# comfy-creator/Comfy-Gen-Server

Hardware: AMD Instinct MI355X
Metric: images/sec (whole node) + sec/image, SDXL 1024 20-step Euler-a at 1/2/4/8 MI355X (higher is better)
Workload: dtype bf16; 1 GPU; model=sdxl-base, global_batch=8, seq_len=16384, resolution=1024, sampler_steps=20, sampler=euler_ancestral, unet_batch_per_gpu=16, parallelism=dp1, pipelined=True

## Files before the change

### comfy_gen_server_amd/_native.py

```python
from __future__ import annotations

import ctypes
import glob
import os
import threading

_HERE = os.path.dirname(os.path.abspath(__file__))
LIB_DIR = os.path.join(_HERE, "lib")
_lock = threading.Lock()
_kernels = None
_kernels_err = None


def kernel_lib_path() -> str:
    return os.environ.get("CGS_KERNELS_SO") or os.path.join(LIB_DIR, "libcgs_kernels.so")


def load_kernels():
    global _kernels, _kernels_err
    if _kernels is not None or _kernels_err is not None:
        return _kernels
    with _lock:
        if _kernels is not None or _kernels_err is not None:
            return _kernels
        path = kernel_lib_path()
        if not os.path.exists(path):
            _kernels_err = f"{path} not built (run python build_native.py)"
            return None
        try:
            import torch
            lib = ctypes.CDLL(path, mode=ctypes.RTLD_GLOBAL)
            _declare(lib)
            _kernels = lib
        except OSError as e:
            _kernels_err = str(e)
            _kernels = None
    return _kernels


def kernels_error():
    return _kernels_err


_P = ctypes.c_void_p
_I = ctypes.c_int
_L = ctypes.c_longlong
_F = ctypes.c_float

KERNEL_SIGNATURES = {
    "cgs_groupnorm_nhwc_ws": [_P, _P, _P, _P, _P, _P, _I, _I, _I, _I, _F, _I, _I, _P],
    "cgs_groupnorm_workspace": [_I, _I, _I],
    "cgs_groupnorm_nhwc_dual": [_P, _P, _I, _P, _P, _P, _P, _P, _I, _I, _I, _I, _F, _I, _I, _P],
    "cgs_layernorm": [_P, _P, _P, _P, _I, _I, _F, _I, _P],
    "cgs_flash_attn_fwd": [_P, _P, _P, _P,
                           _I, _I, _I, _I, _I,
                           _L, _L, _L,
                           _L, _L, _L,
                           _L, _L, _L,
                           _L, _L, _L,
                           _F, _P, _I, _P],
    "cgs_flash_attn_fwd_v": [_P, _P, _P, _P, _I, _I, _I, _I, _I, _L, _L, _L, _L, _L, _L, _L, _L, _L, _L, _L, _L, _F,
                             _I, _P],
    "cgs_flash_attn_fwd_bias": [_P, _P, _P, _P, _I, _I, _I, _I, _I, _L, _L, _L, _L, _L, _L, _L, _L, _L, _L, _L, _L,
                                _F, _P, _P, _I, _P, _P],
    "cgs_flash_attn_fwd_mask": [_P, _P, _P, _P, _I, _I, _I, _I, _I, _L, _L, _L, _L, _L, _L, _L, _L, _L, _L, _L, _L,
                                _F, _P, _I, _L, _L, _L, _P, _I, _P],
    "cgs_flash_attn_fwd_lse": [_P, _P, _P, _P, _P, _I, _I, _I, _I, _I, _L, _L, _L, _L, _L, _L, _L, _L, _L, _L, _L, _L,
                               _F, _P],
    "cgs_gemm_bf16": [_P, _P, _P, _P, _P, _I, _I, _I, _L, _L, _L, _L, _I, _F, _P],
    "cgs_gemm_set_variant": [_I],
    "cgs_conv_set_variant": [_I],
    "cgs_attn_set_variant": [_I],
    "cgs_set_tile_group": [_I],
    "cgs_conv_set_tile_group": [_I],
    "cgs_dwconv_set_px": [_I],
    "cgs_affine_layernorm": [_P, _P, _P, _L, _F, _P, _P, _I, _I, _I, _F, _I, _P],
    "cgs_geglu": [_P, _P, _I, _I, _I, _P],
    "cgs_cfg_combine": [_P, _P, _P, _L, _F, _I, _P],
    "cgs_euler_step": [_P, _P, _P, _L, _F, _F, _F, _P],
    "cgs_timestep_embedding": [_P, _P, _I, _I, _F, _I, _P],
    "cgs_silu": [_P, _P, _L, _I, _P],
    "cgs_act": [_P, _P, _L, _I, _F, _I, _P],
    "cgs_upsample_nearest2x_nhwc": [_P, _P, _I, _I, _I, _I, _I, _P],
    "cgs_dwconv_nhwc": [_P, _P, _P, _P, _I, _I, _I, _I, _I, _I, _I, _P],
    "cgs_dwconv_ln_stats_nhwc": [_P, _P, _P, _P, _P, _I, _I, _I, _I, _I, _I, _F, _I, _P],
    "cgs_conv2d_nhwc": [_P, _P, _P, _P, _P, _I, _I, _I, _I, _I, _I, _I, _I, _I, _I, _I, _P],
    "cgs_fused_bias_act": [_P, _P, _P, _L, _I, _L, _F, _F, _I, _P],
    "cgs_upfirdn2d": [_P, _P, _P, _I, _I, _I, _I, _I, _I, _I, _I, _I, _I, _I, _I, _I, _I, _P],
    "cgs_resize": [_P, _P, _I, _I, _I, _I, _I, _I, _I, _I, _P],
    "cgs_lanczos_u8_h": [_P, _L, _L, _L, _L, _P, _I, _I, _I, _I, _I, _P, _P, _I, _I, _I, _P],
    "cgs_lanczos_u8_v": [_P, _I, _L, _L, _L, _L, _P, _I, _I, _I, _I, _P, _P, _I, _P],
    "cgs_bislerp": [_P, _P, _I, _I, _I, _I, _L, _L, _L, _L, _I, _I, _P, _P, _P, _I, _I, _P],
    "cgs_filter_sep": [_P, _P, _P, _P, _P, _I, _I, _I, _I, _I, _I, _I, _L, _L, _L, _L, _L, _L, _L, _L, _I, _F, _F, _F, _F,
                       _I, _P],
    "cgs_morph_box": [_P, _P, _P, _I, _I, _I, _I, _I, _L, _L, _L, _L, _L, _L, _L, _L, _I, _I, _I, _P],
    "cgs_canny_nms": [_P, _P, _P, _I, _I, _I, _F, _F, _P],
    "cgs_hysteresis_sweep": [_P, _I, _I, _I, _P, _P],
    "cgs_vq_nearest": [_P, _P, _P, _P, _I, _I, _I, _I, _P],
    "cgs_grn_nhwc": [_P, _P, _P, _P, _P, _I, _I, _I, _I, _P],
    "cgs_grn_stats": [_P, _P, _I, _I, _I, _I, _I, _P],
    "cgs_splitk_ws_bytes": [_I, _I, _I],
    "cgs_gemm_bf16_splitk": [_P, _P, _P, _P, _P, _P, _P, _I, _I, _I, _L, _L, _L, _L, _I, _F, _I, _I, _P, _L, _P],
    "cgs_grn_stats_gns": [_P, _P, _I, _I, _I, _P],
    "cgs_grn_apply_gns": [_P, _P, _P, _P, _P, _P, _I, _I, _I, _P],
    "cgs_gemm_bf16_gelu_gns": [_P, _P, _P, _P, _P, _P, _I, _I, _I, _L, _L, _L, _I, _P, _I, _P],
    "cgs_grn_scale_weight": [_P, _P, _P, _I, _I, _I, _I, _P, _P],
    "cgs_h2d_upload": [_P, _P, _L, _L, _I, _P],
    "cgs_gemm_f32": [_P, _P, _P, _P, _P, _I, _I, _I, _L, _L, _L, _L, _I, _F, _I, _I, _L, _L, _L, _P],
    "cgs_conv_f32": [_P, _P, _P, _P, _P, _P, _I, _I, _I, _I, _I, _I, _I, _I, _I, _I, _I, _I, _I, _P],
    "cgs_groupnorm_f32_ws": [_I, _I, _I],
    "cgs_groupnorm_f32": [_P, _P, _I, _P, _P, _P, _P, _P, _I, _I, _I, _I, _F, _I, _P],
    "cgs_layernorm_f32": [_P, _P, _P, _P, _L, _I, _F, _P],
    "cgs_softmax_rows": [_P, _P, _L, _I, _F, _I, _P],
    "cgs_gemm_bf16_w8": [_P, _P, _P, _P, _P, _I, _I, _I, _L, _L, _L, _L, _I, _F, _P],
    "cgs_gemm_bf16_v": [_P, _P, _P, _P, _P, _I, _I, _I, _L, _L, _L, _L, _I, _F, _I, _P],
    "cgs_conv2d_nhwc_v": [_P, _P, _I, _P, _P, _P, _P, _I, _I, _I, _I, _I, _I, _I, _I, _I, _I, _I, _I, _I, _P],
    "cgs_upconv_taps_nhwc": [_P, _P, _P, _P, _I, _I, _I, _I, _I, _P],
    "cgs_conv2d_nhwc_act": [_P, _P, _I, _P, _P, _P, _P, _I, _I, _I, _I, _I, _I, _I, _I, _I, _I, _I, _I, _I, _I, _F,
                            _P],
    "cgs_philox_randn": [_P, _I, _L, ctypes.c_ulonglong, _L, ctypes.c_ulonglong, _P, _F, _I, _P, _P],
    "cgs_euler_ancestral_philox": [_P, _P, _I, _L, _F, _F, _F, ctypes.c_ulonglong, _L, ctypes.c_ulonglong, _P, _P],
    "cgs_brownian_increment": [_P, _I, _L, ctypes.c_ulonglong, _L, ctypes.c_double, ctypes.c_double,
                               ctypes.c_double, ctypes.c_double, ctypes.c_double, _I, _F, _P, _P],
    "cgs_sampler_step_dev": [_P, _P, _P, _P, _I, _L, _F, _P, _I, _P, _P],
    "cgs_step_param": [_P, _I, _P, _I, _I, _P, _P],
    "cgs_step_advance": [_P, _P],
    "cgs_vae_out_u8": [_P, _P, _L, _P],
    "cgs_conv2d_nhwc_ex": [_P, _P, _I, _P, _P, _P, _P, _I, _I, _I, _I, _I, _I, _I, _I, _I, _I, _I, _I, _P],
    "cgs_region_accumulate": [_P, _P, _P, _I, _P, _I, _I, _I, _I, _I, _I, _I, _I, _I, _L, _L, _L, _L, _I, _L, _L,
                              _L, _L, _I, _F, _P],
    "cgs_region_normalize": [_P, _P, _P, _L, _I, _P],
    "cgs_clip_embed": [_P, _P, _P, _P, _I, _I, _I, _I, _I, _P],
    "cgs_pooled_gather": [_P, _P, _P, _I, _I, _I, _I, _P],
    "cgs_layernorm_stats": [_P, _P, _I, _I, _F, _I, _P],
    "cgs_gemm_bf16_lnfold": [_P, _P, _P, _P, _P, _P, _I, _I, _I, _L, _L, _L, _I, _P, _L, _P],
    "cgs_gemm_bf16_lnfold_v": [_P, _P, _P, _P, _P, _P, _I, _I, _I, _L, _L, _L, _I, _P, _L, _I, _P],
    "cgs_v7_ws_bytes": [_I, _I, _I],
    "cgs_v7_set_dbg": [_I],
    "cgs_v6_set_mode": [_I],
    "cgs_attn_set_prio": [_I],
    "cgs_gn_set_blocks": [_I],
    "cgs_conv_smalln_set_lds": [_I],
    "cgs_attn_set_kv2_rows": [_I],
    "cgs_grn_set_rows": [_I],
    "cgs_flash_attn_fwd_ks": [_P, _P, _P, _P, _I, _I, _I, _I, _L, _L, _L, _L, _L, _L, _L, _L, _F, _I, _P, _P, _P],
    "cgs_flash_attn_fwd_kv2": [_P, _P, _P, _P, _P, _P, _I, _I, _I, _I, _I, _L, _L, _L, _L, _L, _L, _L, _L, _L, _L, _L, _L, _F, _P],
    "cgs_conv2d_nhwc_gns": [_P, _P, _I, _P, _P, _P, _P, _I, _I, _I, _I, _I, _I, _I, _I, _I, _I, _I, _I, _P, _P],
    "cgs_groupnorm_band_stats": [_P, _P, _I, _P, _P, _P, _I, _I, _I, _I, _I, _P],
    "cgs_groupnorm_apply_stats": [_P, _P, _I, _P, _P, _P, _P, _P, _P, _I, _I, _I, _I, _I, _I, _P],
    "cgs_groupnorm_nhwc_part": [_P, _P, _P, _P, _P, _P, _P, _I, _I, _I, _I, _I, _F, _I, _I, _P],
    "cgs_groupnorm_nhwc_part_pld": [_P, _P, _P, _P, _P, _I, _P, _P, _I, _I, _I, _I, _I, _F, _I, _I, _P],
    "cgs_groupnorm_nhwc_ws_pld": [_P, _P, _P, _P, _P, _I, _P, _I, _I, _I, _I, _F, _I, _I, _P],
    "cgs_groupnorm_nhwc_dual_pld": [_P, _P, _I, _P, _P, _P, _P, _I, _P, _I, _I, _I, _I, _F, _I, _I, _P],
    "cgs_gemm_bf16_v7ws": [_P, _P, _P, _P, _P, _I, _I, _I, _L, _L, _L, _L, _I, _F, _P, _L, _P],
    "cgs_conv2d_nhwc_v7ws": [_P, _P, _I, _P, _P, _P, _P, _I, _I, _I, _I, _I, _I, _I, _I, _I, _I, _I, _I, _P, _L, _P],
    "cgs_fourier_filter": [_P, _P, _P, _I, _I, _I, _I, _L, _L, _L, _L, _L, _L, _L, _L, _I, _F, _I, _P],
    "cgs_tome_match": [_P, _P, _P, _P, _P, _I, _I, _I, _I, _L, _L, _L, _L, _I, _P],
    "cgs_grn_nhwc_v2": [_P, _P, _P, _P, _P, _I, _I, _I, _I, _I, _P],
    "cgs_grn_slices": [_I, _I, _I],
    "cgs_bgemm_f32": [_P, _P, _P, _I, _I, _I, _I, _L, _L, _L, _L, _L, _L, _L, _L, _F, _I, _I, _P],
    "cgs_softmax2_f32_bf16": [_P, _P, _L, _I, _L, _L, _P],
    "cgs_transpose_bf16": [_P, _P, _I, _I, _L, _L, _P],
    "cgs_abort_stream_capture": [_P],
    "cgs_channel_affine2": [_P, _P, _P, _L, _P, _I, _I, _I, _F, _I, _P],
    "cgs_gemm_bf16_w6": [_P, _P, _P, _P, _P, _P, _P, _I, _I, _I, _L, _L, _L, _L, _I, _F, _I, _I, _I, _I, _P],
    "cgs_gemm_w6_ok": [_I, _I, _I, _L, _L, _L, _L, _I, _I],
    "cgs_gemm_skinny_ws": [_P, _P, _P, _P, _P, _I, _I, _I, _L, _L, _L, _L, _I, _F, _P, _L, _P],
    "cgs_gemm_skinny_ws_bytes": [_I, _I, _I],
    "cgs_gemm_bf16_rowstats": [_P, _P, _P, _P, _P, _I, _I, _I, _L, _L, _L, _L, _I, _F, _P, _P],
    "cgs_gemm_bf16_rowstats_v": [_P, _P, _P, _P, _P, _I, _I, _I, _L, _L, _L, _L, _I, _F, _P, _I, _P],
    "cgs_ln_rs_from_partials": [_P, _P, _I, _I, _F, _P],
    "cgs_conv_v6_set_loader": [_I],
    "cgs_upconv_set_tile_group": [_I],
}


_RESTYPE = {"cgs_groupnorm_workspace": ctypes.c_longlong, "cgs_splitk_ws_bytes": ctypes.c_longlong, "cgs_groupnorm_f32_ws": ctypes.c_longlong, "cgs_grn_slices": ctypes.c_int, "cgs_v7_ws_bytes": ctypes.c_longlong, "cgs_gemm_skinny_ws_bytes": ctypes.c_longlong, "cgs_gemm_set_variant": None, "cgs_v7_set_dbg": None, "cgs_v6_set_mode": None, "cgs_attn_set_prio": None, "cgs_gn_set_blocks": None, "cgs_conv_smalln_set_lds": None, "cgs_attn_set_kv2_rows": None, "cgs_grn_set_rows": None,
            "cgs_conv_set_variant": None, "cgs_set_tile_group": None, "cgs_conv_set_tile_group": None, "cgs_dwconv_set_px": None, "cgs_upconv_set_tile_group": None,
            "cgs_attn_set_variant": None,
            "cgs_conv_v6_set_loader": None}


def _declare(lib):
    for name, argtypes in KERNEL_SIGNATURES.items():
        fn = getattr(lib, name, None)
        if fn is None:
            continue
        fn.argtypes = argtypes
        fn.restype = _RESTYPE.get(name, ctypes.c_int)


def has_kernel(name: str) -> bool:
    lib = load_kernels()
    return lib is not None and getattr(lib, name, None) is not None


_runtime = None
_runtime_err = None


def load_runtime():
    global _runtime, _runtime_err
    if _runtime is not None or _runtime_err is not None:
        return _runtime
    import importlib.util
    import sys
    cands = glob.glob(os.path.join(LIB_DIR, "_cgs_runtime*.so"))
    if not cands:
        _runtime_err = "_cgs_runtime not built"
        return None
    try:
        spec = importlib.util.spec_from_file_location("_cgs_runtime", cands[0])
        mod = importlib.util.module_from_spec(spec)
        spec.loader.exec_module(mod)
        sys.modules["_cgs_runtime"] = mod
        _runtime = mod
    except Exception as e:
        _runtime_err = str(e)
    return _runtime


def runtime_error():
    return _runtime_err
```

### comfy_gen_server_amd/csrc/kernels/norm.hip

```cpp
#include "common.h"

#define GN_THREADS 256
#define GN_MAX_CHUNKS_PER_LANE 4

static int g_gn_blocks = -1;
static int gn_blocks() {
  if (g_gn_blocks < 0) g_gn_blocks = getenv("CGS_GN_BLOCKS") ? atoi(getenv("CGS_GN_BLOCKS")) : 2048;
  return g_gn_blocks > 0 ? g_gn_blocks : 2048;
}
CGS_EXPORT void cgs_gn_set_blocks(int n) { g_gn_blocks = n; }

static inline int gn_pix_per_block(int N, int HW) {
  int target_blocks_per_n = (gn_blocks() + N - 1) / N;
  int ppb = (HW + target_blocks_per_n - 1) / target_blocks_per_n;
  if (ppb < 16) ppb = 16;
  if (N <= 4 && ppb < 64) ppb = 64;
  return ppb;
}

__device__ __forceinline__ const u16* gn_src(const u16* __restrict__ x, const u16* __restrict__ x2, int C, int C1,
                                             size_t pix, int c) {
  return c < C1 ? x + pix * C1 + c : x2 + pix * (size_t)(C - C1) + (c - C1);
}

template <int DT, int KM, int PK = 1>
__global__ __launch_bounds__(GN_THREADS) void gn_partial_kernel(const u16* __restrict__ x, const u16* __restrict__ x2,
                                                               int C1, float* __restrict__ part,
                                                               int HW, int C, int ppb, int nb, int CS) {
  constexpr int GN_UNROLL = 4;
  constexpr int LPG = 64 / PK;
  const int n = blockIdx.y;
  const int blk = blockIdx.x;
  const int c0 = blockIdx.z * CS;
  const int p0 = blk * ppb;
  const int p1 = min(HW, p0 + ppb);
  const int lane = threadIdx.x & 63;
  const int wave = threadIdx.x >> 6;
  const int lch = PK > 1 ? lane % LPG : lane;
  const int pg = PK > 1 ? lane / LPG : 0;
  const int nchunk = CS >> 3;
  const size_t pix0 = (size_t)n * HW;
  float s1[KM][8], s2[KM][8], sh[KM][8];
#pragma unroll
  for (int k = 0; k < KM; ++k) {
    int ch = lch + 64 * k;
    s16x8 v = {};
    if (ch < nchunk && p0 < p1) v = *reinterpret_cast<const s16x8*>(gn_src(x, x2, C, C1, pix0 + p0, c0 + ch * 8));
#pragma unroll
    for (int j = 0; j < 8; ++j) { sh[k][j] = cvt_in<DT>((u16)v[j]); s1[k][j] = 0.f; s2[k][j] = 0.f; }
  }
  int cnt = 0;
  for (int p = p0 + wave * PK + pg; p < p1; p += 4 * PK * GN_UNROLL) {
    s16x8 buf[GN_UNROLL][KM];
#pragma unroll
    for (int u = 0; u < GN_UNROLL; ++u) {
      const int pu = p + 4 * PK * u;
#pragma unroll
      for (int k = 0; k < KM; ++k) {
        int ch = lch + 64 * k;
        if (pu < p1 && ch < nchunk) buf[u][k] = *reinterpret_cast<const s16x8*>(gn_src(x, x2, C, C1, pix0 + pu, c0 + ch * 8));
      }
    }
#pragma unroll
    for (int u = 0; u < GN_UNROLL; ++u) {
      if (p + 4 * PK * u < p1) {
        cnt++;
#pragma unroll
        for (int k = 0; k < KM; ++k) {
          if (lch + 64 * k < nchunk) {
#pragma unroll
            for (int j = 0; j < 8; ++j) {
              float d = cvt_in<DT>((u16)buf[u][k][j]) - sh[k][j];
              s1[k][j] += d;
              s2[k][j] += d * d;
            }
          }
        }
      }
    }
  }
  if constexpr (PK > 1) {
#pragma unroll
    for (int off = LPG; off < 64; off <<= 1) {
      cnt += __shfl_xor(cnt, off);
#pragma unroll
      for (int j = 0; j < 8; ++j) {
        s1[0][j] += __shfl_xor(s1[0][j], off);
        s2[0][j] += __shfl_xor(s2[0][j], off);
      }
    }
  }
  extern __shared__ __attribute__((aligned(16))) float gn_smem[];
  float* lmean = gn_smem;
  float* lm2 = gn_smem + 4 * CS;
  __shared__ int lcnt[4];
  if (lane == 0) lcnt[wave] = cnt;
#pragma unroll
  for (int k = 0; k < KM; ++k) {
    int ch = lch + 64 * k;
    if (ch < nchunk && pg == 0) {
#pragma unroll
      for (int j = 0; j < 8; ++j) {
        float m = 0.f, m2 = 0.f;
        if (cnt > 0) {
          m = sh[k][j] + s1[k][j] / cnt;
          m2 = fmaxf(0.f, s2[k][j] - s1[k][j] * s1[k][j] / cnt);
        }
        lmean[wave * CS + ch * 8 + j] = m;
        lm2[wave * CS + ch * 8 + j] = m2;
      }
    }
  }
  __syncthreads();
  for (int c = threadIdx.x; c < CS; c += GN_THREADS) {
    float n_a = 0.f, mean = 0.f, m2 = 0.f;
    for (int w = 0; w < 4; ++w) {
      float n_b = (float)lcnt[w];
      if (n_b <= 0.f) continue;
      float mb = lmean[w * CS + c], m2b = lm2[w * CS + c];
      float nn = n_a + n_b;
      float d = mb - mean;
      mean += d * n_b / nn;
      m2 += m2b + d * d * n_a * n_b / nn;
      n_a = nn;
    }
    size_t o = (((size_t)n * nb + blk) * C + c0 + c) * 2;
    part[o] = mean;
    part[o + 1] = m2;
  }
}

__device__ __forceinline__ void chan_merge(float& na, float& ma, float& qa, float nb, float mb, float qb) {
  const float nn = na + nb;
  if (nn <= 0.f) return;
  const float d = mb - ma;
  const float f = nb / nn;
  ma += d * f;
  qa += qb + d * d * na * f;
  na = nn;
}

template <bool STATS_ONLY = false>
__global__ __launch_bounds__(256) void gn_finalize_kernel(const float* __restrict__ part, const void* __restrict__ gamma,
                                                         const void* __restrict__ beta, const void* __restrict__ pre_add,
                                                         float* __restrict__ ab, int HW, int C, int G, int ppb, int nb,
                                                         float eps, int wdt, int pld) {
  const int g = blockIdx.x;
  const int n = blockIdx.y;
  const int tid = threadIdx.x;
  const int Cg = C / G;
  const int items = Cg * nb;
  __shared__ float red[3][4];
  auto chan_shift = [&](int c) -> float {
    if (!pre_add) return 0.f;
    const size_t i = (size_t)n * pld + c;
    return (wdt == CGS_BF16) ? bf2f(((const u16*)pre_add)[i])
                             : (wdt == CGS_F16 ? h2f(((const u16*)pre_add)[i]) : ((const float*)pre_add)[i]);
  };
  float cnt = 0.f, mean = 0.f, m2 = 0.f;
  constexpr int U = 8;
  for (int it0 = tid; it0 < items; it0 += 256 * U) {
    float2 v[U];
    float nbv[U];
#pragma unroll
    for (int u = 0; u < U; ++u) {
      const int it = it0 + 256 * u;
      v[u] = make_float2(0.f, 0.f);
      nbv[u] = 0.f;
      if (it < items) {
        const int b = it / Cg, cc = it - b * Cg;
        const int c = g * Cg + cc;
        v[u] = *reinterpret_cast<const float2*>(part + (((size_t)n * nb + b) * C + c) * 2);
        v[u].x += chan_shift(c);
        nbv[u] = (float)(min(HW, b * ppb + ppb) - b * ppb);
      }
    }
#pragma unroll
    for (int u = 0; u < U; ++u) chan_merge(cnt, mean, m2, nbv[u], v[u].x, v[u].y);
  }
#pragma unroll
  for (int off = 32; off > 0; off >>= 1) {
    const float on = __shfl_xor(cnt, off), om = __shfl_xor(mean, off), oq = __shfl_xor(m2, off);
    chan_merge(cnt, mean, m2, on, om, oq);
  }
  if ((tid & 63) == 0) { red[0][tid >> 6] = cnt; red[1][tid >> 6] = mean; red[2][tid >> 6] = m2; }
  __syncthreads();
  cnt = red[0][0]; mean = red[1][0]; m2 = red[2][0];
#pragma unroll
  for (int w = 1; w < 4; ++w) chan_merge(cnt, mean, m2, red[0][w], red[1][w], red[2][w]);
  if constexpr (STATS_ONLY) {
    if (tid == 0) {
      ab[((size_t)n * G + g) * 2] = mean;
      ab[((size_t)n * G + g) * 2 + 1] = m2;
    }
    return;
  }
  const float var = m2 / fmaxf(cnt, 1.f);
  const float rstd = rsqrtf(fmaxf(var, 0.f) + eps);
  for (int cc = tid; cc < Cg; cc += 256) {
    int c = g * Cg + cc;
    float gm = 1.f, bt = 0.f;
    if (gamma) gm = (wdt == CGS_BF16) ? bf2f(((const u16*)gamma)[c]) : (wdt == CGS_F16 ? h2f(((const u16*)gamma)[c]) : ((const float*)gamma)[c]);
    if (beta) bt = (wdt == CGS_BF16) ? bf2f(((const u16*)beta)[c]) : (wdt == CGS_F16 ? h2f(((const u16*)beta)[c]) : ((const float*)beta)[c]);
    float a = rstd * gm;
    ab[((size_t)n * C + c) * 2] = a;
    ab[((size_t)n * C + c) * 2 + 1] = (chan_shift(c) - mean) * a + bt;
  }
}

template <int DT, bool SILU>
__global__ __launch_bounds__(256) void gn_apply_kernel(const u16* __restrict__ x, const u16* __restrict__ x2, int C1,
                                                      u16* __restrict__ y,
                                                      const float* __restrict__ ab, int rows_total, int rows_per_iter,
                                                      int HW, int C) {
  const int cpr = C >> 3;
  const int tid = blockIdx.x * blockDim.x + threadIdx.x;
  if (tid >= rows_per_iter * cpr) return;
  const int ch = tid % cpr;
  int cur_n = -1;
  float a[8], bb[8];
  auto coef = [&](int n) {
    if (n != cur_n) {
      cur_n = n;
      const float4* abp = reinterpret_cast<const float4*>(ab + ((size_t)n * C + ch * 8) * 2);
#pragma unroll
      for (int j = 0; j < 4; ++j) {
        float4 t = abp[j];
        a[2 * j] = t.x; bb[2 * j] = t.y; a[2 * j + 1] = t.z; bb[2 * j + 1] = t.w;
      }
    }
  };
  auto apply = [&](int row, const s16x8& v) {
    coef(row / HW);
    s16x8 o;
#pragma unroll
    for (int j = 0; j < 8; ++j) {
      float f = cvt_in<DT>((u16)v[j]) * a[j] + bb[j];
      if (SILU) f = silu_f(f);
      o[j] = (short)cvt_out<DT>(f);
    }
    reinterpret_cast<s16x8*>(y)[(size_t)row * cpr + ch] = o;
  };
  int row = tid / cpr;
  for (; row + rows_per_iter < rows_total; row += 2 * rows_per_iter) {
    const s16x8 v0 = *reinterpret_cast<const s16x8*>(gn_src(x, x2, C, C1, (size_t)row, ch * 8));
    const s16x8 v1 = *reinterpret_cast<const s16x8*>(gn_src(x, x2, C, C1, (size_t)(row + rows_per_iter), ch * 8));
    apply(row, v0);
    apply(row + rows_per_iter, v1);
  }
  if (row < rows_total) apply(row, *reinterpret_cast<const s16x8*>(gn_src(x, x2, C, C1, (size_t)row, ch * 8)));
}

template <int PV>
__global__ __launch_bounds__(256) void ln_rs_from_partials_kernel(const float* __restrict__ part, float* __restrict__ rs,
                                                                  int M, int P, float eps) {
  const int row = blockIdx.x * 256 + threadIdx.x;
  if (row >= M) return;
  float n, mean, m2;
  auto chan = [&](float vm, float vq) {
    const float nn = n + 80.f, d = vm - mean, f = 80.f / nn;
    mean += d * f;
    m2 += vq + d * d * n * f;
    n = nn;
  };
  if constexpr (PV > 0) {
    const float4* p = reinterpret_cast<const float4*>(part) + (long long)row * (P >> 1);
    float4 v[PV];
#pragma unroll
    for (int c = 0; c < PV; ++c) v[c] = 2 * c < P ? p[c] : float4{0.f, 0.f, 0.f, 0.f};
    n = 80.f, mean = v[0].x, m2 = v[0].y;
    chan(v[0].z, v[0].w);
#pragma unroll
    for (int c = 1; c < PV; ++c)
      if (2 * c < P) {
        chan(v[c].x, v[c].y);
        chan(v[c].z, v[c].w);
      }
  } else {
    const float2* p = reinterpret_cast<const float2*>(part) + (long long)row * P;
    n = 80.f, mean = p[0].x, m2 = p[0].y;
    for (int c = 1; c < P; ++c) chan(p[c].x, p[c].y);
  }
  reinterpret_cast<float2*>(rs)[row] = float2{mean, rsqrtf(m2 / n + eps)};
}

CGS_EXPORT int cgs_ln_rs_from_partials(const float* part, float* rs, int M, int P, float eps, hipStream_t stream) {
  if (M <= 0 || P <= 0) return (int)hipErrorInvalidValue;
  const unsigned grid = (unsigned)((M + 255) / 256);
  const bool vec = P % 2 == 0 && ((uintptr_t)part & 15) == 0;
  if (vec && P <= 8) ln_rs_from_partials_kernel<4><<<grid, 256, 0, stream>>>(part, rs, M, P, eps);
  else if (vec && P <= 16) ln_rs_from_partials_kernel<8><<<grid, 256, 0, stream>>>(part, rs, M, P, eps);
  else ln_rs_from_partials_kernel<0><<<grid, 256, 0, stream>>>(part, rs, M, P, eps);
  return (int)hipGetLastError();
}

CGS_EXPORT long long cgs_groupnorm_workspace(int N, int HW, int C) {
  int ppb = gn_pix_per_block(N, HW);
  int nb = (HW + ppb - 1) / ppb;
  return (long long)N * nb * C * 2 * 4 + (long long)N * C * 2 * 4 + 256;
}

static int gn_apply_launch(const void* x, const void* x2, int C1, void* y, const float* ab, int N, int HW, int C,
                           int silu, int dtype, hipStream_t stream);

static int gn_slices(int C) {
  const int ns0 = (C + 2047) / 2048;
  if (C > 512 && C <= 1024 && C % 16 == 0) return 2;
  if (C <= 1024 || C % 8) return ns0;
  const int tot = C / 8;
  int best = ns0;
  float bu = -1.f;
  for (int ns = (C + 511) / 512; ns <= tot; ++ns) {
    if (tot % ns) continue;
    const int nch = tot / ns;
    const int lanes = nch <= 8 ? 8 : nch <= 16 ? 16 : nch <= 32 ? 32 : 64;
    const float u = (float)nch / (float)lanes;
    if (u >= 0.9f) return ns;
    if (u > bu) { bu = u; best = ns; }
  }
  return best;
}

using GnPartialKernel = decltype(&gn_partial_kernel<CGS_BF16, 1>);
template <int DT>
static GnPartialKernel gn_partial_kernel_for(int nch) {
  if (nch <= 8) return gn_partial_kernel<DT, 1, 8>;
  if (nch <= 16) return gn_partial_kernel<DT, 1, 4>;
  if (nch <= 32) return gn_partial_kernel<DT, 1, 2>;
  if (nch <= 64) return gn_partial_kernel<DT, 1>;
  if (nch <= 128) return gn_partial_kernel<DT, 2>;
  if (nch <= 192) return gn_partial_kernel<DT, 3>;
  return gn_partial_kernel<DT, 4>;
}

static int gn_partial_launch(const void* x, const void* x2, int C1, float* part, int N, int HW, int C, int G, int dtype,
                             hipStream_t stream, int* ppb, int* nb) {
  const int ns = gn_slices(C);
  if (C % 8 || C % G || C % (8 * ns) || C > 8192 || C1 % 8 || C1 > C) return (int)hipErrorInvalidValue;
  const int CS = C / ns;
  *ppb = gn_pix_per_block(N, HW);
  *nb = (HW + *ppb - 1) / *ppb;
  const GnPartialKernel kern =
      dtype == CGS_BF16 ? gn_partial_kernel_for<CGS_BF16>(CS / 8) : gn_partial_kernel_for<CGS_F16>(CS / 8);
  kern<<<dim3(*nb, N, ns), GN_THREADS, 8 * CS * sizeof(float), stream>>>((const u16*)x, (const u16*)x2, C1, part, HW, C,
                                                                         *ppb, *nb, CS);
  return 0;
}

static int groupnorm_impl(const void* x, const void* x2, int C1, void* y, const void* gamma, const void* beta,
                          const void* pre_add, void* ws, int N, int HW, int C, int G, float eps, int silu, int dtype,
                          hipStream_t stream, int pld) {
  if (pre_add && pld < C) return (int)hipErrorInvalidValue;
  int ppb, nb;
  float* part = (float*)ws;
  if (const int rc = gn_partial_launch(x, x2, C1, part, N, HW, C, G, dtype, stream, &ppb, &nb)) return rc;
  float* ab = part + (size_t)N * nb * C * 2;
  gn_finalize_kernel<<<dim3(G, N), 256, 0, stream>>>(part, gamma, beta, pre_add, ab, HW, C, G, ppb, nb, eps, dtype,
                                                    pld);
  return gn_apply_launch(x, x2, C1, y, ab, N, HW, C, silu, dtype, stream);
}

static int groupnorm_stats_impl(const void* x, const void* x2, int C1, const void* pre_add, void* ws, float* stats,
                                int N, int HW, int C, int G, int dtype, hipStream_t stream) {
  int ppb, nb;
  float* part = (float*)ws;
  if (const int rc = gn_partial_launch(x, x2, C1, part, N, HW, C, G, dtype, stream, &ppb, &nb)) return rc;
  gn_finalize_kernel<true><<<dim3(G, N), 256, 0, stream>>>(part, nullptr, nullptr, pre_add, stats, HW, C, G, ppb, nb,
                                                          0.f, dtype, C);
  return (int)hipGetLastError();
}

__global__ __launch_bounds__(256) void gn_ab_from_stats_kernel(const float* __restrict__ mr, const void* __restrict__ gamma,
                                                               const void* __restrict__ beta,
                                                               const void* __restrict__ pre_add, float* __restrict__ ab,
                                                               int N, int C, int G, int wdt) {
  const int i = blockIdx.x * 256 + threadIdx.x;
  if (i >= N * C) return;
  const int n = i / C, c = i - n * C, g = c / (C / G);
  auto ld = [&](const void* p, int idx) -> float {
    return (wdt == CGS_BF16) ? bf2f(((const u16*)p)[idx]) : (wdt == CGS_F16 ? h2f(((const u16*)p)[idx]) : ((const float*)p)[idx]);
  };
  const float mean = mr[((size_t)n * G + g) * 2], rstd = mr[((size_t)n * G + g) * 2 + 1];
  const float gm = gamma ? ld(gamma, c) : 1.f, bt = beta ? ld(beta, c) : 0.f;
  const float sh = pre_add ? ld(pre_add, n * C + c) : 0.f;
  const float a = rstd * gm;
  ab[(size_t)i * 2] = a;
  ab[(size_t)i * 2 + 1] = (sh - mean) * a + bt;
}

CGS_EXPORT int cgs_groupnorm_band_stats(const void* x, const void* x2, int C1, const void* pre_add, void* ws,
                                        float* stats, int N, int HW, int C, int G, int dtype, hipStream_t stream) {
  if (!stats || !ws || HW <= 0) return (int)hipErrorInvalidValue;
  return groupnorm_stats_impl(x, x2 ? x2 : nullptr, x2 ? C1 : C, pre_add, ws, stats, N, HW, C, G, dtype, stream);
}

CGS_EXPORT int cgs_groupnorm_apply_stats(const void* x, const void* x2, int C1, void* y, const void* gamma,
                                         const void* beta, const void* pre_add, const float* mean_rstd, float* ab,
                                         int N, int HW, int C, int G, int silu, int dtype, hipStream_t stream) {
  if (C % 8 || C % G || !mean_rstd || !ab || (x2 && (C1 % 8 || C1 > C))) return (int)hipErrorInvalidValue;
  gn_ab_from_stats_kernel<<<(unsigned)((N * C + 255) / 256), 256, 0, stream>>>(mean_rstd, gamma, beta, pre_add, ab, N,
                                                                              C, G, dtype);
  return gn_apply_launch(x, x2, x2 ? C1 : C, y, ab, N, HW, C, silu, dtype, stream);
}

static int gn_apply_launch(const void* x, const void* x2, int C1, void* y, const float* ab, int N, int HW, int C,
                           int silu, int dtype, hipStream_t stream) {
  const int cpr = C / 8;
  const long long rows_total = (long long)N * HW;
  if (rows_total == 0) return (int)hipGetLastError();
  if (rows_total * cpr >= (1LL << 31)) return (int)hipErrorInvalidValue;
  long long chunks = rows_total * cpr;
  long long nbk = (chunks + 255) / 256;
  int blocks = (int)(nbk < 8192 ? nbk : 8192);
  int rows_per_iter = (blocks * 256) / cpr;
  if (rows_per_iter < 1) rows_per_iter = 1, blocks = (cpr + 255) / 256;
  if (dtype == CGS_BF16) {
    if (silu) gn_apply_kernel<CGS_BF16, true><<<blocks, 256, 0, stream>>>((const u16*)x, (const u16*)x2, C1, (u16*)y, ab, (int)rows_total, rows_per_iter, HW, C);
    else gn_apply_kernel<CGS_BF16, false><<<blocks, 256, 0, stream>>>((const u16*)x, (const u16*)x2, C1, (u16*)y, ab, (int)rows_total, rows_per_iter, HW, C);
  } else {
    if (silu) gn_apply_kernel<CGS_F16, true><<<blocks, 256, 0, stream>>>((const u16*)x, (const u16*)x2, C1, (u16*)y, ab, (int)rows_total, rows_per_iter, HW, C);
    else gn_apply_kernel<CGS_F16, false><<<blocks, 256, 0, stream>>>((const u16*)x, (const u16*)x2, C1, (u16*)y, ab, (int)rows_total, rows_per_iter, HW, C);
  }
  return (int)hipGetLastError();
}

static int groupnorm_part_impl(const void* x, void* y, const void* gamma, const void* beta, const void* pre_add,
                               int pld, const float* part, float* ab, int N, int HW, int C, int G, int ppb, float eps,
                               int silu, int dtype, hipStream_t stream) {
  if (C % 8 || C % G || ppb <= 0 || HW % ppb || !part || !ab || (pre_add && pld < C)) return (int)hipErrorInvalidValue;
  const int nb = HW / ppb;
  gn_finalize_kernel<<<dim3(G, N), 256, 0, stream>>>(part, gamma, beta, pre_add, ab, HW, C, G, ppb, nb, eps, dtype,
                                                    pld);
  return gn_apply_launch(x, nullptr, C, y, ab, N, HW, C, silu, dtype, stream);
}

CGS_EXPORT int cgs_groupnorm_nhwc_part(const void* x, void* y, const void* gamma, const void* beta, const void* pre_add,
                                       const float* part, float* ab, int N, int HW, int C, int G, int ppb, float eps,
                                       int silu, int dtype, hipStream_t stream) {
  return groupnorm_part_impl(x, y, gamma, beta, pre_add, C, part, ab, N, HW, C, G, ppb, eps, silu, dtype, stream);
}

CGS_EXPORT int cgs_groupnorm_nhwc_ws(const void* x, void* y, const void* gamma, const void* beta, const void* pre_add,
                                     void* ws, int N, int HW, int C, int G, float eps, int silu, int dtype,
                                     hipStream_t stream) {
  return groupnorm_impl(x, nullptr, C, y, gamma, beta, pre_add, ws, N, HW, C, G, eps, silu, dtype, stream, C);
}

CGS_EXPORT int cgs_groupnorm_nhwc_dual(const void* x, const void* x2, int C1, void* y, const void* gamma,
                                       const void* beta, const void* pre_add, void* ws, int N, int HW, int C, int G,
                                       float eps, int silu, int dtype, hipStream_t stream) {
  return groupnorm_impl(x, x2, C1, y, gamma, beta, pre_add, ws, N, HW, C, G, eps, silu, dtype, stream, C);
}

CGS_EXPORT int cgs_groupnorm_nhwc_ws_pld(const void* x, void* y, const void* gamma, const void* beta,
                                         const void* pre_add, int pld, void* ws, int N, int HW, int C, int G, float eps,
                                         int silu, int dtype, hipStream_t stream) {
  return groupnorm_impl(x, nullptr, C, y, gamma, beta, pre_add, ws, N, HW, C, G, eps, silu, dtype, stream, pld);
}

CGS_EXPORT int cgs_groupnorm_nhwc_dual_pld(const void* x, const void* x2, int C1, void* y, const void* gamma,
                                           const void* beta, const void* pre_add, int pld, void* ws, int N, int HW,
                                           int C, int G, float eps, int silu, int dtype, hipStream_t stream) {
  return groupnorm_impl(x, x2, C1, y, gamma, beta, pre_add, ws, N, HW, C, G, eps, silu, dtype, stream, pld);
}

CGS_EXPORT int cgs_groupnorm_nhwc_part_pld(const void* x, void* y, const void* gamma, const void* beta,
                                           const void* pre_add, int pld, const float* part, float* ab, int N, int HW,
                                           int C, int G, int ppb, float eps, int silu, int dtype, hipStream_t stream) {
  return groupnorm_part_impl(x, y, gamma, beta, pre_add, pld, part, ab, N, HW, C, G, ppb, eps, silu, dtype, stream);
}

#define LN_MAXK 8

template <int LPR>
__device__ __forceinline__ float group_sum(float v) {
#pragma unroll
  for (int o = LPR / 2; o > 0; o >>= 1) v += __shfl_xor(v, o, 64);
  return v;
}

template <int DT, int LPR>
__global__ __launch_bounds__(256) void layernorm_kernel(const u16* __restrict__ x, u16* __restrict__ y,
                                                       const u16* __restrict__ w, const u16* __restrict__ b, int rows,
                                                       int C, float eps) {
  constexpr int RPB = 256 / LPR;
  const int lane = threadIdx.x % LPR;
  const int row = blockIdx.x * RPB + threadIdx.x / LPR;
  const bool live = row < rows;
  const int nch = C >> 3;
  const u16* xr = x + (size_t)(live ? row : 0) * C;
  float v[LN_MAXK][8];
  float s = 0.f;
#pragma unroll
  for (int k = 0; k < LN_MAXK; ++k) {
    int ch = lane + LPR * k;
    if (live && ch < nch) {
      s16x8 t = reinterpret_cast<const s16x8*>(xr)[ch];
#pragma unroll
      for (int j = 0; j < 8; ++j) { v[k][j] = cvt_in<DT>((u16)t[j]); s += v[k][j]; }
    }
  }
  float mean = group_sum<LPR>(s) / C;
  float q = 0.f;
#pragma unroll
  for (int k = 0; k < LN_MAXK; ++k) {
    int ch = lane + LPR * k;
    if (live && ch < nch) {
#pragma unroll
      for (int j = 0; j < 8; ++j) { float d = v[k][j] - mean; q += d * d; }
    }
  }
  float rstd = rsqrtf(group_sum<LPR>(q) / C + eps);
  if (!live) return;
  u16* yr = y + (size_t)row * C;
#pragma unroll
  for (int k = 0; k < LN_MAXK; ++k) {
    int ch = lane + LPR * k;
    if (ch < nch) {
      s16x8 wv, bv;
      if (w) wv = reinterpret_cast<const s16x8*>(w)[ch];
      if (b) bv = reinterpret_cast<const s16x8*>(b)[ch];
      s16x8 o;
#pragma unroll
      for (int j = 0; j < 8; ++j) {
        float f = (v[k][j] - mean) * rstd * (w ? cvt_in<DT>((u16)wv[j]) : 1.f) + (b ? cvt_in<DT>((u16)bv[j]) : 0.f);
        o[j] = (short)cvt_out<DT>(f);
      }
      reinterpret_cast<s16x8*>(yr)[ch] = o;
    }
  }
}


template <int DT, int LPR>
__global__ __launch_bounds__(256) void affine_layernorm_kernel(const u16* __restrict__ x, const u16* __restrict__ sc,
                                                               const u16* __restrict__ sh, long long ld, float add,
                                                               u16* __restrict__ xa, u16* __restrict__ y, int rows,
                                                               int HW, int C, float eps) {
  constexpr int RPB = 256 / LPR;
  const int lane = threadIdx.x % LPR;
  const int row = blockIdx.x * RPB + threadIdx.x / LPR;
  const bool live = row < rows;
  const int nch = C >> 3;
  const size_t ro = (size_t)(live ? row : 0) * C;
  const long long n = (live ? row : 0) / HW;
  float v[LN_MAXK][8];
  float s = 0.f;
#pragma unroll
  for (int k = 0; k < LN_MAXK; ++k) {
    const int ch = lane + LPR * k;
    if (live && ch < nch) {
      const s16x8 t = reinterpret_cast<const s16x8*>(x + ro)[ch];
      const s16x8 a = *reinterpret_cast<const s16x8*>(sc + n * ld + ch * 8);
      const s16x8 b = *reinterpret_cast<const s16x8*>(sh + n * ld + ch * 8);
      s16x8 o;
#pragma unroll
      for (int j = 0; j < 8; ++j) {
        o[j] = (short)cvt_out<DT>(__builtin_fmaf(cvt_in<DT>((u16)t[j]), add + cvt_in<DT>((u16)a[j]), cvt_in<DT>((u16)b[j])));
        v[k][j] = cvt_in<DT>((u16)o[j]);
        s += v[k][j];
      }
      reinterpret_cast<s16x8*>(xa + ro)[ch] = o;
    }
  }
  const float mean = group_sum<LPR>(s) / C;
  float q = 0.f;
#pragma unroll
  for (int k = 0; k < LN_MAXK; ++k) {
    const int ch = lane + LPR * k;
    if (live && ch < nch) {
#pragma unroll
      for (int j = 0; j < 8; ++j) { const float d = v[k][j] - mean; q += d * d; }
    }
  }
  const float rstd = rsqrtf(group_sum<LPR>(q) / C + eps);
  if (!live) return;
#pragma unroll
  for (int k = 0; k < LN_MAXK; ++k) {
    const int ch = lane + LPR * k;
    if (ch < nch) {
      s16x8 o;
#pragma unroll
      for (int j = 0; j < 8; ++j) o[j] = (short)cvt_out<DT>((v[k][j] - mean) * rstd);
      reinterpret_cast<s16x8*>(y + ro)[ch] = o;
    }
  }
}

CGS_EXPORT int cgs_affine_layernorm(const void* x, const void* scale, const void* shift, long long ld, float add,
                                    void* xa, void* y, int N, int HW, int C, float eps, int dtype,
                                    hipStream_t stream) {
  if (N <= 0 || HW <= 0) return 0;
  const int nch = C / 8;
  if (C % 8 || ld % 8 || nch > 64 * LN_MAXK || dtype == CGS_F32 ||
      (((uintptr_t)x | (uintptr_t)xa | (uintptr_t)y | (uintptr_t)scale | (uintptr_t)shift) & 15))
    return (int)hipErrorInvalidValue;
  const long long rows = (long long)N * HW;
  if (rows >= (1LL << 31)) return (int)hipErrorInvalidValue;
  const int lpr = nch <= 8 * LN_MAXK ? 8 : nch <= 16 * LN_MAXK ? 16 : nch <= 32 * LN_MAXK ? 32 : 64;
  const dim3 grid((unsigned)((rows + 256 / lpr - 1) / (256 / lpr)));
#define CGS_ALN(L)                                                                                                  \
  if (dtype == CGS_BF16)                                                                                            \
    affine_layernorm_kernel<CGS_BF16, L><<<grid, 256, 0, stream>>>((const u16*)x, (const u16*)scale, (const u16*)shift, \
                                                                   ld, add, (u16*)xa, (u16*)y, (int)rows, HW, C, eps); \
  else                                                                                                              \
    affine_layernorm_kernel<CGS_F16, L><<<grid, 256, 0, stream>>>((const u16*)x, (const u16*)scale, (const u16*)shift, \
                                                                  ld, add, (u16*)xa, (u16*)y, (int)rows, HW, C, eps);
  if (lpr == 8) { CGS_ALN(8) } else if (lpr == 16) { CGS_ALN(16) } else if (lpr == 32) { CGS_ALN(32) } else { CGS_ALN(64) }
#undef CGS_ALN
  return (int)hipGetLastError();
}

template <int DT, int LPR>
__global__ __launch_bounds__(256) void ln_stats_kernel(const u16* __restrict__ x, float* __restrict__ rs, int rows,
                                                      int C, float eps) {
  constexpr int RPB = 256 / LPR;
  const int lane = threadIdx.x % LPR;
  const int row = blockIdx.x * RPB + threadIdx.x / LPR;
  const bool live = row < rows;
  const int nch = C >> 3;
  const u16* xr = x + (size_t)(live ? row : 0) * C;
  float v[LN_MAXK][8];
  float s = 0.f;
#pragma unroll
  for (int k = 0; k < LN_MAXK; ++k) {
    int ch = lane + LPR * k;
    if (live && ch < nch) {
      s16x8 t = reinterpret_cast<const s16x8*>(xr)[ch];
#pragma unroll
      for (int j = 0; j < 8; ++j) { v[k][j] = cvt_in<DT>((u16)t[j]); s += v[k][j]; }
    }
  }
  const float mean = group_sum<LPR>(s) / C;
  float q = 0.f;
#pragma unroll
  for (int k = 0; k < LN_MAXK; ++k) {
    int ch = lane + LPR * k;
    if (live && ch < nch) {
#pragma unroll
      for (int j = 0; j < 8; ++j) { float d = v[k][j] - mean; q += d * d; }
    }
  }
  const float rstd = rsqrtf(group_sum<LPR>(q) / C + eps);
  if (live && lane == 0) reinterpret_cast<float2*>(rs)[row] = float2{mean, rstd};
// ... 170 lines not shown
```

Measured before the change: 3.498 images/s.

## Restructure GroupNorm partial-stats kernel: deeper load pipelining, geometry-aligned blocks, coalesced finalize

Reworks the GroupNorm partial statistics kernel. It precomputes per-chunk source pointers, unrolls deeper (8 rows in flight when each lane holds one chunk), and drops per-iteration bounds checks by using a masked tail. Block geometry now counts channel slices and rounds pixels-per-block to the unroll trip, with the default block target halved. The finalize kernel gives each thread one channel and strides over blocks for more coalesced reads, and the slice heuristic is tweaked. The deeper unroll raises register pressure, and fewer blocks could reduce occupancy on small layers.

```diff
diff --git a/comfy_gen_server_amd/_native.py b/comfy_gen_server_amd/_native.py
--- a/comfy_gen_server_amd/_native.py
+++ b/comfy_gen_server_amd/_native.py
@@ -158,6 +158,8 @@
     "cgs_tome_match": [_P, _P, _P, _P, _P, _I, _I, _I, _I, _L, _L, _L, _L, _I, _P],
     "cgs_grn_nhwc_v2": [_P, _P, _P, _P, _P, _I, _I, _I, _I, _I, _P],
     "cgs_grn_slices": [_I, _I, _I],
+    "cgs_gn_slices": [_I],
+    "cgs_gn_stat_ppb": [_I, _I, _I],
     "cgs_bgemm_f32": [_P, _P, _P, _I, _I, _I, _I, _L, _L, _L, _L, _L, _L, _L, _L, _F, _I, _I, _P],
     "cgs_softmax2_f32_bf16": [_P, _P, _L, _I, _L, _L, _P],
     "cgs_transpose_bf16": [_P, _P, _I, _I, _L, _L, _P],
diff --git a/comfy_gen_server_amd/csrc/kernels/norm.hip b/comfy_gen_server_amd/csrc/kernels/norm.hip
--- a/comfy_gen_server_amd/csrc/kernels/norm.hip
+++ b/comfy_gen_server_amd/csrc/kernels/norm.hip
@@ -2,33 +2,32 @@
 
 #define GN_THREADS 256
 #define GN_MAX_CHUNKS_PER_LANE 4
-
+#ifndef GN_ROWS_IN_FLIGHT
+#define GN_ROWS_IN_FLIGHT 8
+#endif
+
+#define GN_BLOCKS_DEFAULT 1024
 static int g_gn_blocks = -1;
 static int gn_blocks() {
-  if (g_gn_blocks < 0) g_gn_blocks = getenv("CGS_GN_BLOCKS") ? atoi(getenv("CGS_GN_BLOCKS")) : 2048;
-  return g_gn_blocks > 0 ? g_gn_blocks : 2048;
-}
-CGS_EXPORT void cgs_gn_set_blocks(int n) { g_gn_blocks = n; }
-
-static inline int gn_pix_per_block(int N, int HW) {
-  int target_blocks_per_n = (gn_blocks() + N - 1) / N;
-  int ppb = (HW + target_blocks_per_n - 1) / target_blocks_per_n;
-  if (ppb < 16) ppb = 16;
-  if (N <= 4 && ppb < 64) ppb = 64;
-  return ppb;
-}
+  if (g_gn_blocks < 0) g_gn_blocks = getenv("CGS_GN_BLOCKS") ? atoi(getenv("CGS_GN_BLOCKS")) : 0;
+  return g_gn_blocks > 0 ? g_gn_blocks : GN_BLOCKS_DEFAULT;
+}
+CGS_EXPORT void cgs_gn_set_blocks(int n) { g_gn_blocks = n > 0 ? n : 0; }
 
 __device__ __forceinline__ const u16* gn_src(const u16* __restrict__ x, const u16* __restrict__ x2, int C, int C1,
                                              size_t pix, int c) {
   return c < C1 ? x + pix * C1 + c : x2 + pix * (size_t)(C - C1) + (c - C1);
 }
+
+__host__ __device__ constexpr int gn_unroll(int KM) { return KM == 1 ? GN_ROWS_IN_FLIGHT : KM == 2 ? 4 : 2; }
 
 template <int DT, int KM, int PK = 1>
 __global__ __launch_bounds__(GN_THREADS) void gn_partial_kernel(const u16* __restrict__ x, const u16* __restrict__ x2,
                                                                int C1, float* __restrict__ part,
                                                                int HW, int C, int ppb, int nb, int CS) {
-  constexpr int GN_UNROLL = 4;
+  constexpr int U = gn_unroll(KM);
   constexpr int LPG = 64 / PK;
+  constexpr int SPAN = 4 * PK;
   const int n = blockIdx.y;
   const int blk = blockIdx.x;
   const int c0 = blockIdx.z * CS;
@@ -39,43 +38,59 @@
   const int lch = PK > 1 ? lane % LPG : lane;
   const int pg = PK > 1 ? lane / LPG : 0;
   const int nchunk = CS >> 3;
-  const size_t pix0 = (size_t)n * HW;
+  const u16* src[KM];
+  int ld[KM];
+  bool act[KM];
   float s1[KM][8], s2[KM][8], sh[KM][8];
 #pragma unroll
   for (int k = 0; k < KM; ++k) {
-    int ch = lch + 64 * k;
-    s16x8 v = {};
-    if (ch < nchunk && p0 < p1) v = *reinterpret_cast<const s16x8*>(gn_src(x, x2, C, C1, pix0 + p0, c0 + ch * 8));
+    const int ch = lch + 64 * k;
+    act[k] = ch < nchunk;
+    const int c = c0 + (act[k] ? ch : ch % nchunk) * 8;
+    ld[k] = c < C1 ? C1 : C - C1;
+    src[k] = (c < C1 ? x + c : x2 + (c - C1)) + (size_t)n * HW * ld[k];
+    const s16x8 v = *reinterpret_cast<const s16x8*>(src[k] + (size_t)p0 * ld[k]);
 #pragma unroll
     for (int j = 0; j < 8; ++j) { sh[k][j] = cvt_in<DT>((u16)v[j]); s1[k][j] = 0.f; s2[k][j] = 0.f; }
   }
-  int cnt = 0;
-  for (int p = p0 + wave * PK + pg; p < p1; p += 4 * PK * GN_UNROLL) {
-    s16x8 buf[GN_UNROLL][KM];
-#pragma unroll
-    for (int u = 0; u < GN_UNROLL; ++u) {
-      const int pu = p + 4 * PK * u;
-#pragma unroll
-      for (int k = 0; k < KM; ++k) {
-        int ch = lch + 64 * k;
-        if (pu < p1 && ch < nchunk) buf[u][k] = *reinterpret_cast<const s16x8*>(gn_src(x, x2, C, C1, pix0 + pu, c0 + ch * 8));
-      }
-    }
-#pragma unroll
-    for (int u = 0; u < GN_UNROLL; ++u) {
-      if (p + 4 * PK * u < p1) {
-        cnt++;
-#pragma unroll
-        for (int k = 0; k < KM; ++k) {
-          if (lch + 64 * k < nchunk) {
-#pragma unroll
-            for (int j = 0; j < 8; ++j) {
-              float d = cvt_in<DT>((u16)buf[u][k][j]) - sh[k][j];
-              s1[k][j] += d;
-              s2[k][j] += d * d;
-            }
-          }
-        }
+  auto accum = [&](int k, const s16x8& v, float w) {
+#pragma unroll
+    for (int j = 0; j < 8; ++j) {
+      const float d = (cvt_in<DT>((u16)v[j]) - sh[k][j]) * w;
+      s1[k][j] += d;
+      s2[k][j] += d * d;
+    }
+  };
+  int p = p0 + wave * PK + pg;
+  int cnt = p < p1 ? (p1 - p + SPAN - 1) / SPAN : 0;
+  if (act[0]) {
+    for (; p + SPAN * (U - 1) < p1; p += SPAN * U) {
+      s16x8 buf[U][KM];
+#pragma unroll
+      for (int u = 0; u < U; ++u) {
+#pragma unroll
+        for (int k = 0; k < KM; ++k)
+          buf[u][k] = *reinterpret_cast<const s16x8*>(src[k] + (size_t)(p + SPAN * u) * ld[k]);
+      }
+#pragma unroll
+      for (int u = 0; u < U; ++u) {
+#pragma unroll
+        for (int k = 0; k < KM; ++k) accum(k, buf[u][k], 1.f);
+      }
+    }
+    if (p < p1) {
+      s16x8 buf[U - 1][KM];
+#pragma unroll
+      for (int u = 0; u < U - 1; ++u) {
+#pragma unroll
+        for (int k = 0; k < KM; ++k)
+          buf[u][k] = *reinterpret_cast<const s16x8*>(src[k] + (size_t)min(p + SPAN * u, p1 - 1) * ld[k]);
+      }
+#pragma unroll
+      for (int u = 0; u < U - 1; ++u) {
+        const float w = p + SPAN * u < p1 ? 1.f : 0.f;
+#pragma unroll
+        for (int k = 0; k < KM; ++k) accum(k, buf[u][k], w);
       }
     }
   }
@@ -95,25 +110,29 @@
   float* lm2 = gn_smem + 4 * CS;
   __shared__ int lcnt[4];
   if (lane == 0) lcnt[wave] = cnt;
+  const float inv = cnt > 0 ? 1.f / (float)cnt : 0.f;
 #pragma unroll
   for (int k = 0; k < KM; ++k) {
-    int ch = lch + 64 * k;
-    if (ch < nchunk && pg == 0) {
+    const int ch = lch + 64 * k;
+    if (act[k] && pg == 0) {
+      float m[8], q[8];
 #pragma unroll
       for (int j = 0; j < 8; ++j) {
-        float m = 0.f, m2 = 0.f;
-        if (cnt > 0) {
-          m = sh[k][j] + s1[k][j] / cnt;
-          m2 = fmaxf(0.f, s2[k][j] - s1[k][j] * s1[k][j] / cnt);
-        }
-        lmean[wave * CS + ch * 8 + j] = m;
-        lm2[wave * CS + ch * 8 + j] = m2;
-      }
+        m[j] = cnt > 0 ? sh[k][j] + s1[k][j] * inv : 0.f;
+        q[j] = fmaxf(0.f, s2[k][j] - s1[k][j] * s1[k][j] * inv);
+      }
+      float4* dm = reinterpret_cast<float4*>(lmean + wave * CS + ch * 8);
+      float4* dq = reinterpret_cast<float4*>(lm2 + wave * CS + ch * 8);
+      dm[0] = make_float4(m[0], m[1], m[2], m[3]);
+      dm[1] = make_float4(m[4], m[5], m[6], m[7]);
+      dq[0] = make_float4(q[0], q[1], q[2], q[3]);
+      dq[1] = make_float4(q[4], q[5], q[6], q[7]);
     }
   }
   __syncthreads();
   for (int c = threadIdx.x; c < CS; c += GN_THREADS) {
     float n_a = 0.f, mean = 0.f, m2 = 0.f;
+#pragma unroll
     for (int w = 0; w < 4; ++w) {
       float n_b = (float)lcnt[w];
       if (n_b <= 0.f) continue;
@@ -124,9 +143,7 @@
       m2 += m2b + d * d * n_a * n_b / nn;
       n_a = nn;
     }
-    size_t o = (((size_t)n * nb + blk) * C + c0 + c) * 2;
-    part[o] = mean;
-    part[o + 1] = m2;
+    *reinterpret_cast<float2*>(part + (((size_t)n * nb + blk) * C + c0 + c) * 2) = make_float2(mean, m2);
   }
 }
 
@@ -149,7 +166,6 @@
   const int n = blockIdx.y;
   const int tid = threadIdx.x;
   const int Cg = C / G;
-  const int items = Cg * nb;
   __shared__ float red[3][4];
   auto chan_shift = [&](int c) -> float {
     if (!pre_add) return 0.f;
@@ -159,24 +175,28 @@
   };
   float cnt = 0.f, mean = 0.f, m2 = 0.f;
   constexpr int U = 8;
-  for (int it0 = tid; it0 < items; it0 += 256 * U) {
-    float2 v[U];
-    float nbv[U];
-#pragma unroll
-    for (int u = 0; u < U; ++u) {
-      const int it = it0 + 256 * u;
-      v[u] = make_float2(0.f, 0.f);
-      nbv[u] = 0.f;
-      if (it < items) {
-        const int b = it / Cg, cc = it - b * Cg;
-        const int c = g * Cg + cc;
-        v[u] = *reinterpret_cast<const float2*>(part + (((size_t)n * nb + b) * C + c) * 2);
-        v[u].x += chan_shift(c);
-        nbv[u] = (float)(min(HW, b * ppb + ppb) - b * ppb);
-      }
-    }
-#pragma unroll
-    for (int u = 0; u < U; ++u) chan_merge(cnt, mean, m2, nbv[u], v[u].x, v[u].y);
+  const int TB = Cg >= 256 ? 1 : 256 / Cg;
+  const int bl = Cg >= 256 ? 0 : tid / Cg;
+  if (bl < TB) {
+    for (int cc = Cg >= 256 ? tid : tid - bl * Cg; cc < Cg; cc += 256) {
+      const int c = g * Cg + cc;
+      const float shift = chan_shift(c);
+      const float* pp = part + ((size_t)n * nb * C + c) * 2;
+      for (int b0 = bl; b0 < nb; b0 += TB * U) {
+        float2 v[U];
+        float nbv[U];
+#pragma unroll
+        for (int u = 0; u < U; ++u) {
+          const bool ok = b0 + TB * u < nb;
+          const int b = ok ? b0 + TB * u : nb - 1;
+          const float2 t = *reinterpret_cast<const float2*>(pp + (size_t)b * C * 2);
+          v[u] = ok ? t : make_float2(0.f, 0.f);
+          nbv[u] = ok ? (float)(min(HW, b * ppb + ppb) - b * ppb) : 0.f;
+        }
+#pragma unroll
+        for (int u = 0; u < U; ++u) chan_merge(cnt, mean, m2, nbv[u], v[u].x + shift, v[u].y);
+      }
+    }
   }
 #pragma unroll
   for (int off = 32; off > 0; off >>= 1) {
@@ -294,10 +314,36 @@
   return (int)hipGetLastError();
 }
 
+static int gn_slices(int C);
+
+struct GnGeom { int ns, CS, ppb, nb; };
+
+static GnGeom gn_geometry(int N, int HW, int C) {
+  GnGeom g;
+  g.ns = gn_slices(C);
+  g.CS = C / g.ns;
+  const int nch = (g.CS + 7) / 8;
+  const int pk = nch <= 8 ? 8 : nch <= 16 ? 4 : nch <= 32 ? 2 : 1;
+  const int km = nch <= 64 ? 1 : nch <= 128 ? 2 : nch <= 192 ? 3 : 4;
+  const int trip = 4 * pk * gn_unroll(km);
+  const long long per_n = (gn_blocks() + (long long)N * g.ns - 1) / ((long long)N * g.ns);
+  const int raw = (int)((HW + per_n - 1) / per_n);
+  g.ppb = raw / trip * trip;
+  if (g.ppb < trip) g.ppb = trip;
+  if (N <= 4 && g.ppb < 64) g.ppb = 64;
+  g.nb = (HW + g.ppb - 1) / g.ppb;
+  return g;
+}
+
 CGS_EXPORT long long cgs_groupnorm_workspace(int N, int HW, int C) {
-  int ppb = gn_pix_per_block(N, HW);
-  int nb = (HW + ppb - 1) / ppb;
-  return (long long)N * nb * C * 2 * 4 + (long long)N * C * 2 * 4 + 256;
+  if (N <= 0 || HW <= 0 || C <= 0) return 256;
+  const GnGeom g = gn_geometry(N, HW, C);
+  return (long long)N * g.nb * C * 2 * 4 + (long long)N * C * 2 * 4 + 256;
+}
+
+CGS_EXPORT int cgs_gn_slices(int C) { return C > 0 ? gn_slices(C) : 0; }
+CGS_EXPORT int cgs_gn_stat_ppb(int N, int HW, int C) {
+  return N > 0 && HW > 0 && C > 0 ? gn_geometry(N, HW, C).ppb : 0;
 }
 
 static int gn_apply_launch(const void* x, const void* x2, int C1, void* y, const float* ab, int N, int HW, int C,
@@ -308,11 +354,13 @@
   if (C > 512 && C <= 1024 && C % 16 == 0) return 2;
   if (C <= 1024 || C % 8) return ns0;
   const int tot = C / 8;
+  const int nch0 = tot / ns0;
   int best = ns0;
-  float bu = -1.f;
+  float bu = tot % ns0 ? -1.f : (float)nch0 / (float)(64 * ((nch0 + 63) / 64));
   for (int ns = (C + 511) / 512; ns <= tot; ++ns) {
     if (tot % ns) continue;
     const int nch = tot / ns;
+    if (nch < 8 && bu >= 0.f) break;
     const int lanes = nch <= 8 ? 8 : nch <= 16 ? 16 : nch <= 32 ? 32 : 64;
     const float u = (float)nch / (float)lanes;
     if (u >= 0.9f) return ns;
@@ -335,11 +383,12 @@
 
 static int gn_partial_launch(const void* x, const void* x2, int C1, float* part, int N, int HW, int C, int G, int dtype,
                              hipStream_t stream, int* ppb, int* nb) {
-  const int ns = gn_slices(C);
+  if (N <= 0 || HW <= 0 || C <= 0 || G <= 0) return (int)hipErrorInvalidValue;
+  const GnGeom g = gn_geometry(N, HW, C);
+  const int ns = g.ns, CS = g.CS;
   if (C % 8 || C % G || C % (8 * ns) || C > 8192 || C1 % 8 || C1 > C) return (int)hipErrorInvalidValue;
-  const int CS = C / ns;
-  *ppb = gn_pix_per_block(N, HW);
-  *nb = (HW + *ppb - 1) / *ppb;
+  *ppb = g.ppb;
+  *nb = g.nb;
   const GnPartialKernel kern =
       dtype == CGS_BF16 ? gn_partial_kernel_for<CGS_BF16>(CS / 8) : gn_partial_kernel_for<CGS_F16>(CS / 8);
   kern<<<dim3(*nb, N, ns), GN_THREADS, 8 * CS * sizeof(float), stream>>>((const u16*)x, (const u16*)x2, C1, part, HW, C,
```

After: 3.516 images/s (median of 6 runs). About the same (+0.5%).
